# EpicOne1/grad_traj_optimization

Hardware: AMD Instinct MI355X
Metric: cost+grad evals/sec (batched trajectories) (higher is better)
Workload: dtype f64

## Files before the change

### grad_traj_optimization_amd/csrc/gtop_kernels.hip

```cpp

#include "gtop_wave_kernel.h"

#ifdef GTOP_CONSISTENT_TU
template <typename MM> using GtopModeOf = GtopConsistent<MM>;
#define GTOP_LAUNCHER(name) name##_consistent
constexpr bool kReferenceObject = false;
#else
template <typename MM> using GtopModeOf = MM;
#define GTOP_LAUNCHER(name) name
constexpr bool kReferenceObject = true;
#endif

namespace {

constexpr int kWaveMinw3From = 3072;

template <typename R, typename MM>
using WaveKernelFn = void (*)(const R *, const R *, const R *, const R *, int, int, int, int, int, int,
                              const GtopKernelArgs<R>, const GtopWaveConsts<R>, const MM, const GtopSetupConsts<R>);

template <typename R, bool WIDE, int SPL, int NT, int MINW, typename MM, bool LONG, int NW = 1>
static WaveKernelFn<R, MM> pick_body(bool colli, bool dyn) {
  if (!colli) {
    if constexpr (kIsCons<MM>) return nullptr;
    else return gtop_eval_wave_kernel<R, WIDE, SPL, NT, false, MINW, MM, false, LONG, NW>;
  }
  if (dyn) return gtop_eval_wave_kernel<R, WIDE, SPL, NT, true, (MINW < 3 ? 3 : MINW), MM, true, LONG, NW>;
  return gtop_eval_wave_kernel<R, WIDE, SPL, NT, true, MINW, MM, false, LONG, NW>;
}

template <typename R, bool WIDE, typename MM>
static WaveKernelFn<R, MM> pick_geometry(const GtopEvalPlan &p, int B, bool colli, bool dyn) {
  constexpr bool MMA = kIsMma<MM>;
  if (p.is_long) return pick_body<R, WIDE, 6, 1, 3, MM, true>(colli, dyn);
  if (p.spl == 30) {
    if constexpr (MMA) return nullptr;
    else return pick_body<R, WIDE, 30, 1, 3, MM, false>(colli, dyn);
  }
  if (p.spl == 10) {
    if constexpr (MMA) return nullptr;
    else return pick_body<R, WIDE, 10, 1, 3, MM, false>(colli, dyn);
  }
  if constexpr (!MMA) {
    if (p.nw == 2) return pick_body<R, WIDE, 3, 1, 2, MM, false, 2>(colli, dyn);
  }
  if (p.spl == 3) {
    if constexpr (!MMA && !(WIDE && sizeof(R) == 8)) {
      if (B >= kWaveMinw3From) return pick_body<R, WIDE, 3, 1, 3, MM, false>(colli, dyn);
    }
    return pick_body<R, WIDE, 3, 1, 2, MM, false>(colli, dyn);
  }
  if (p.nt == 2) {
    if constexpr (MMA) {
      if (dyn) return nullptr;
      if constexpr (kIsCons<MM>) {
        return colli ? gtop_eval_wave_kernel<R, WIDE, 6, 2, true, 3, MM, false, false, 1> : nullptr;
      } else {
        return colli ? gtop_eval_wave_kernel<R, WIDE, 6, 2, true, 3, MM, false, false, 1>
                     : gtop_eval_wave_kernel<R, WIDE, 6, 2, false, 3, MM, false, false, 1>;
      }
    } else {
      return pick_body<R, WIDE, 6, 2, 3, MM, false>(colli, dyn);
    }
  }
  return pick_body<R, WIDE, 6, 1, 3, MM, false>(colli, dyn);
}

template <bool WIDE, int SPL, int NT, typename MM, bool LONG>
static WaveKernelFn<double, MM> pick_body_moving(bool dyn) {
  if (dyn) return gtop_eval_wave_kernel<double, WIDE, SPL, NT, true, 3, MM, true, LONG, 1>;
  return gtop_eval_wave_kernel<double, WIDE, SPL, NT, true, 3, MM, false, LONG, 1>;
// ... 20 lines not shown
template <typename R> static bool has_collision_term(const GtopKernelArgs<R> &args) {
  return !((args.wc < (R)0 ? -args.wc : args.wc) < (R)1e-4);
}
template <typename MM> static GtopModeOf<MM> mode_args(const MM &st) {
  GtopModeOf<MM> w;
  static_cast<MM &>(w) = st;
  return w;
}

template <typename R, typename MM>
static hipError_t launch_wave(const GtopKernelArgs<R> &args, const MM &st, const GtopEvalPlan &plan, bool dyn,
                              hipStream_t stream) {
  constexpr bool MMA = kIsMma<MM>;
  constexpr bool MOV = kIsMov<MM>;
  if (args.B <= 0) return hipSuccess;
  GtopKernelArgs<R> wa = args;
  if (wa.step == 1) wa.ws = (R)0;
  const bool colli = has_collision_term(wa);
  dyn = dyn && wa.step == 2;
  const bool wide = !gtop_field_is_narrow(wa.nx, wa.ny, wa.nz, sizeof(R));
  WaveKernelFn<R, MM> kern;
  if constexpr (MOV) {
    if constexpr (!kIsCons<MM>) {
      using Base = typename MovingBase<MM>::type;
      if (!colli) return launch_wave<R, Base>(args, static_cast<const Base &>(st), plan, dyn, stream);
    }
    kern = wide ? pick_geometry_moving<true, MM>(plan, dyn) : pick_geometry_moving<false, MM>(plan, dyn);
  } else if constexpr (MMA && sizeof(R) == 4) {
    if (wide) return hipErrorInvalidValue;
    kern = pick_geometry<R, false, MM>(plan, wa.B, colli, dyn);
  } else {
    kern = wide ? pick_geometry<R, true, MM>(plan, wa.B, colli, dyn) : pick_geometry<R, false, MM>(plan, wa.B, colli, dyn);
  }
  if (!kern) return hipErrorInvalidValue;
  const size_t smem = gtop_wave_lds_bytes(plan, wa.m, MMA ? sizeof(double) : sizeof(R), MMA);
  if (smem > 160u * 1024u) return hipErrorInvalidValue;
  if (smem > 64u * 1024u) {
    hipError_t e = hipFuncSetAttribute(reinterpret_cast<const void *>(kern), hipFuncAttributeMaxDynamicSharedMemorySize,
                                       (int)smem);
    if (e != hipSuccess) return e;
  }
  const int n = 9 * (wa.m - 1);
  const long long per_launch = (long long)kMaxGroupsPerLaunch * plan.nt;
  if (MMA && wa.B > per_launch) return hipErrorInvalidValue;
  for (long long b0 = 0; b0 < args.B; b0 += per_launch) {
    GtopKernelArgs<R> s = wa;
    s.B = (int)((args.B - b0) < per_launch ? (args.B - b0) : per_launch);
    s.x = wa.x + (size_t)b0 * n;
    s.Df = wa.Df + (size_t)b0 * 18;
    s.T = wa.T + (size_t)b0 * wa.t_stride;
    s.cost = wa.cost ? wa.cost + b0 : nullptr;
    s.grad = wa.grad ? wa.grad + (size_t)b0 * n : nullptr;
    const int groups = (s.B + plan.nt - 1) / plan.nt;
    const int grid = 8 * ((groups + 7) / 8);
    MM sst = st;
    if constexpr (MOV) {
      if (sst.mk.t0) sst.mk.t0 += (size_t)b0 * (size_t)sst.mk.t0_stride;
    }
    hipLaunchKernelGGL(kern, dim3(grid), dim3(64 * plan.nw), smem, stream, s.x, s.Df, s.T, s.sdf, s.B, s.m, s.t_stride, s.nx, s.ny,
                       s.nz, s, GtopWaveConsts<R>{}, sst, GtopSetupConsts<R>{});
    hipError_t e = hipGetLastError();
    if (e != hipSuccess) return e;
  }
  return hipSuccess;
}

}


template <typename R>
hipError_t GTOP_LAUNCHER(gtop_launch_eval)(const GtopKernelArgs<R> &args, const GtopEvalPlan &plan, bool dyn, hipStream_t stream) {
  if (kReferenceObject && plan.consistent && has_collision_term(args)) return gtop_launch_eval_consistent<R>(args, plan, dyn, stream);
  return launch_wave<R, GtopModeOf<GtopNoMma>>(args, mode_args(GtopNoMma{}), plan, dyn, stream);
}

template <template <typename> class Moving = GtopMoving, typename Base>
static Moving<Base> moving_kernel_args(const Base &st, const GtopMovingArgs &mov) {
  Moving<Base> mm;
  static_cast<Base &>(mm) = st;
  mm.mk = GtopMovK{mov.rows, mov.t0, mov.nbox, mov.t0_stride};
  return mm;
}
hipError_t GTOP_LAUNCHER(gtop_launch_eval_moving)(const GtopKernelArgs<double> &args, const GtopEvalPlan &plan, bool dyn,
                                                  const GtopMovingArgs &mov, hipStream_t stream) {
  if (!mov.rows || mov.nbox < 1 || mov.nbox > GTOP_MOVING_MAX_BOXES) return hipErrorInvalidValue;
  if (kReferenceObject && plan.consistent && has_collision_term(args)) return gtop_launch_eval_moving_consistent(args, plan, dyn, mov, stream);
  if (mov.poly)
    return launch_wave<double, GtopModeOf<GtopMovingPoly<GtopNoMma>>>(args, mode_args(moving_kernel_args<GtopMovingPoly>(GtopNoMma{}, mov)), plan, dyn, stream);
  return launch_wave<double, GtopModeOf<GtopMoving<GtopNoMma>>>(args, mode_args(moving_kernel_args(GtopNoMma{}, mov)), plan, dyn, stream);
}
hipError_t GTOP_LAUNCHER(gtop_launch_eval_mma_moving)(const GtopKernelArgs<double> &args, const GtopMmaState &st,
                                                      const GtopEvalPlan &plan, bool dyn, const GtopMovingArgs &mov,
                                                      hipStream_t stream) {
  if (!mov.rows || mov.nbox < 1 || mov.nbox > GTOP_MOVING_MAX_BOXES) return hipErrorInvalidValue;
  if (plan.nt != 1) return hipErrorInvalidValue;
  if (kReferenceObject && plan.consistent && has_collision_term(args)) return gtop_launch_eval_mma_moving_consistent(args, st, plan, dyn, mov, stream);
  if (mov.poly)
    return launch_wave<double, GtopModeOf<GtopMovingPoly<GtopMmaState>>>(args, mode_args(moving_kernel_args<GtopMovingPoly>(st, mov)), plan, dyn, stream);
  return launch_wave<double, GtopModeOf<GtopMoving<GtopMmaState>>>(args, mode_args(moving_kernel_args(st, mov)), plan, dyn, stream);
}

hipError_t GTOP_LAUNCHER(gtop_launch_eval_mma)(const GtopKernelArgs<double> &args, const GtopMmaState &st,
                                               const GtopEvalPlan &plan, bool dyn, hipStream_t stream) {
  if (plan.nw != 1 || plan.spl == 30 || plan.spl == 10 || (plan.nt != 1 && !(plan.nt == 2 && plan.spl == 6 && !plan.is_long))) return hipErrorInvalidValue;
  if (kReferenceObject && plan.consistent && has_collision_term(args)) return gtop_launch_eval_mma_consistent(args, st, plan, dyn, stream);
  return launch_wave<double, GtopModeOf<GtopMmaState>>(args, mode_args(st), plan, dyn, stream);
}
hipError_t GTOP_LAUNCHER(gtop_launch_eval_mma)(const GtopKernelArgs<float> &args, const GtopMmaState &st,
                                               const GtopEvalPlan &plan, bool dyn, hipStream_t stream) {
  if (plan.nw != 1 || plan.spl == 30 || plan.spl == 10 || (plan.nt != 1 && !(plan.nt == 2 && plan.spl == 6 && !plan.is_long))) return hipErrorInvalidValue;
  if (kReferenceObject && plan.consistent && has_collision_term(args)) return gtop_launch_eval_mma_consistent(args, st, plan, dyn, stream);
  return launch_wave<float, GtopModeOf<GtopMmaState>>(args, mode_args(st), plan, dyn, stream);
}
// ... 27 lines not shown
```

### grad_traj_optimization_amd/csrc/gtop_wave_kernel.h

```cpp
#ifndef GTOP_WAVE_KERNEL_H_
#define GTOP_WAVE_KERNEL_H_
#include <type_traits>

#include "gtop_device_common.h"
#include "gtop_edt_lookup.h"
#include "gtop_kernels.h"

namespace {

#if defined(GTOP_STAMPS) && defined(GTOP_CONSISTENT_TU)
#undef GTOP_STAMPS
#endif
#ifdef GTOP_STAMPS
__device__ unsigned long long g_gtop_stamps[4096][16];
#if GTOP_STAMPS == 2
#define GTOP_STAMP_WANTED(i) ((i) == 0 || (i) == 11)
#else
#define GTOP_STAMP_WANTED(i) true
#endif
#define GTOP_STAMP(i)                                                                          \
  do {                                                                                         \
    if (GTOP_STAMP_WANTED(i)) {                                                                \
      unsigned long long t_;                                                                   \
      __builtin_amdgcn_sched_barrier(0);                                                       \
// ... 484 lines not shown
    q[k][4] = (K.k7 * V - K.k15 * P - A) * iT4;
    q[k][5] = (K.k6 * P - K.k3 * V + (C)0.5 * A) * iT5;
  }
}

template <typename C>
__device__ __forceinline__ C gtop_jerk_term(const C (&q)[3][6], C T, C wj, const GtopWaveConsts<C> &K, C (&g)[3][3]) {
  const C T2 = T * T, T3 = T2 * T, T4 = T2 * T2, T5 = T4 * T;
  const C Q33 = K.q36 * T, Q34 = K.q72 * T2, Q35 = K.q120 * T3, Q44 = K.q192 * T3, Q45 = K.q360 * T4, Q55 = K.q720 * T5;
  const C wj2 = wj + wj;
  C jc = (C)0;
#pragma unroll
  for (int k = 0; k < 3; ++k) {
    const C c3 = q[k][3], c4 = q[k][4], c5 = q[k][5];
    const C q3 = Q33 * c3 + Q34 * c4 + Q35 * c5;
    const C q4 = Q34 * c3 + Q44 * c4 + Q45 * c5;
    const C q5 = Q35 * c3 + Q45 * c4 + Q55 * c5;
    jc += c3 * q3 + c4 * q4 + c5 * q5;
    g[k][0] = wj2 * q3; g[k][1] = wj2 * q4; g[k][2] = wj2 * q5;
  }
  return wj * jc;
}

struct GtopNoMma {};
template <typename Base> struct GtopMoving : Base {
  GtopMovK mk;
};
template <typename Base> struct GtopMovingPoly : Base {
  GtopMovK mk;
};
template <typename MM> constexpr bool kIsMov = false;
template <typename Base> constexpr bool kIsMov<GtopMoving<Base>> = true;
template <typename Base> constexpr bool kIsMov<GtopMovingPoly<Base>> = true;
template <typename MM> constexpr bool kIsMovPoly = false;
template <typename Base> constexpr bool kIsMovPoly<GtopMovingPoly<Base>> = true;
template <typename MM> constexpr bool kIsMma = std::is_base_of<GtopMmaState, MM>::value;
template <typename Base> struct GtopConsistent : Base {};
template <typename MM> constexpr bool kIsCons = false;
template <typename Base> constexpr bool kIsCons<GtopConsistent<Base>> = true;
template <typename Base> constexpr bool kIsMov<GtopConsistent<Base>> = kIsMov<Base>;
template <typename Base> constexpr bool kIsMovPoly<GtopConsistent<Base>> = kIsMovPoly<Base>;
template <typename R, bool WIDE, typename MM, int SPL, int MINW, bool DYN, bool LONG>
constexpr int gtop_wave_budget() {
  if (kIsCons<MM> && kIsMovPoly<MM> && kIsMma<MM> && DYN && SPL == 6 && !LONG) return 1;
  return ((kIsMma<MM> && SPL == 6) || DYN || kIsMov<MM> || ((WIDE || LONG) && sizeof(R) == 8 && SPL >= 6) ||
          (sizeof(R) == 4 && SPL >= 6))
             ? 2
             : MINW;
}

template <typename R, bool WIDE, int SPL, int NT, bool COLLI, int MINW, typename MM = GtopNoMma, bool DYN = false,
          bool LONG = false, int NW = 1>
__global__ void __launch_bounds__(64 * NW) __attribute__((amdgpu_waves_per_eu(gtop_wave_budget<R, WIDE, MM, SPL, MINW, DYN, LONG>())))
gtop_eval_wave_kernel(const R *__restrict__ arg_x, const R *__restrict__ arg_Df, const R *__restrict__ arg_T,
                      const R *__restrict__ arg_sdf, int arg_B, int arg_m, int arg_t_stride, int arg_nx, int arg_ny,
                      int arg_nz, const GtopKernelArgs<R> arg_rest, const GtopWaveConsts<R> K, const MM st,
                      const GtopSetupConsts<R> KD) {
  constexpr bool MMA = kIsMma<MM>;
  constexpr bool MOV = kIsMov<MM>;
  constexpr bool CONS = kIsCons<MM>;
  static_assert(!CONS || COLLI, "the consistent gradient differs in the sample loop only");
  static_assert(!MMA || NT == 1 || (SPL == 6 && !LONG), "the optimizer loop: one trajectory per wavefront, or two at five lanes per segment");
  using In = typename std::conditional<MMA, double, R>::type;
  GtopKernelArgs<R> a = arg_rest;
  a.x = arg_x; a.Df = arg_Df; a.T = arg_T; a.sdf = arg_sdf;
  a.B = arg_B; a.m = arg_m; a.t_stride = arg_t_stride;
  a.nx = arg_nx; a.ny = arg_ny; a.nz = arg_nz;
  constexpr int LPS = kSamples / SPL;
  constexpr int SPW = 64 / LPS;
  constexpr int kStride = gtop_tile_stride(SPL, NW);
  constexpr int kMVc = gtop_mma_rows(SPL, NT);
  static_assert(SPL == 3 || SPL == 6 || SPL == 10 || SPL == 30, "10 or 5 lanes per segment; three or one with as many trajectories per wavefront as fit");
  constexpr bool MANY = SPL == 30 || SPL == 10;
  static_assert(!MANY || (NT == 1 && !LONG && !MMA && NW == 1 && MINW >= 3), "one lane per segment: plain evaluation, one sample (pair) at a time");
  static_assert(SPL == 3 || MINW >= 3, "six samples per lane: one (pair) at a time only");
  static_assert(NT == 1 || NT == 2, "one or two trajectories per wavefront");
  static_assert(!LONG || (SPL == 6 && NT == 1), "more than 12 segments: five lanes per segment, one trajectory");
  static_assert(!DYN || (COLLI && MINW >= 3), "the velocity/acceleration block lives in the sample loop, one sample at a time");
  static_assert(NW == 1 || (NW == 2 && SPL == 3 && NT == 1 && !LONG && !MMA), "two wavefronts per trajectory: plain evaluation at ten lanes per segment");
  static_assert(!MOV || (COLLI && MINW >= 3 && !kIsF32<R> && (SPL == 3 || SPL == 6) && NW == 1),
                "the moving-obstacle term: fp64, in the sample loop, one sample at a time, ten or five lanes per segment");
  extern __shared__ __align__(16) unsigned char smem_raw[];
  R *tile = reinterpret_cast<R *>(smem_raw);
  GTOP_STAMP(0);
  GTOP_STAMP_HWID();
  const int lane = NW == 2 ? (int)(threadIdx.x & 63u) : (int)threadIdx.x;
  const int wave = NW == 2 ? (int)(threadIdx.x >> 6) : 0;
  const int m = a.m, ndp = 3 * m - 3, n = 3 * ndp;
  if constexpr (LONG) __builtin_assume(m > SPW);
  else __builtin_assume(m >= 2 && NT * m <= NW * SPW);
  __builtin_assume(lane >= 0 && lane < 64);
  const int tstride = LONG ? gtop_tile_stride_long(m) : kStride;
  const int kMV = LONG ? gtop_mma_rows_long(n) : kMVc;
  const int nchunks = LONG ? (m + SPW - 1) / SPW : 1;
  constexpr int kTileRows = gtop_tile_rows(LONG);
  GTOP_STAMP(1);

  const int nt = MANY ? SPW / m : NT;
  const int ngroups = (a.B + nt - 1) / nt;
  const int per_xcd = (ngroups + 7) >> 3;
  const int grp_raw = ((int)blockIdx.x & 7) * per_xcd + ((int)blockIdx.x >> 3);
  const bool grp_ok = grp_raw < ngroups;
  const int grp = grp_ok ? grp_raw : ngroups - 1;
  const int b0 = grp * nt;

  const int slot_w = lane / LPS, li = lane - slot_w * LPS;
  const int slot = wave * SPW + slot_w;
  int tl = 0, s = slot;
  if constexpr (MANY) {
    tl = (int)(((unsigned)slot * (unsigned)((65536 + m - 1) / m)) >> 16);
    s -= tl * m;
  } else if constexpr (NT == 2) {
    tl = s >= m;
    s -= tl * m;
  }
  bool seg_ok = grp_ok & (slot_w < SPW) & (slot < nt * m) & (b0 + tl < a.B);
  if (!seg_ok) { tl = 0; s = 0; }

  unsigned long long t_launch = 0ull;
  int npass = 1;
  if constexpr (MMA) {
    t_launch = wall_clock64();
    npass = st.iters;
  }
  [[maybe_unused]] double *mv = nullptr;
  [[maybe_unused]] const int kState = LONG ? 0 : gtop_state_doubles(false, kMVc, 0);
  [[maybe_unused]] GtopMmaVecs mvecs[NT] = {};
  [[maybe_unused]] GtopMmaScalars msc[NT] = {};
  [[maybe_unused]] bool mma_live[NT] = {};
  if constexpr (MMA) {
    mv = reinterpret_cast<double *>(tile) + kTileRows * tstride + gtop_grad_rows(LONG, kMV);
#pragma unroll
    for (int t = 0; t < NT; ++t) {
    double *mvt = mv + t * kState;
    const int bt = b0 + t;
    mvecs[t] = GtopMmaVecs{mvt, mvt + kMV, mvt + 2 * kMV, mvt + 3 * kMV, mvt + 4 * kMV, mvt + 5 * kMV, mvt + 6 * kMV,
                           mvt + 7 * kMV, mvt + kMV};
    mma_live[t] = grp_ok & (bt < a.B);
    if (mma_live[t]) {
      const size_t o = (size_t)bt * n;
      const double *Df64 = reinterpret_cast<const double *>(a.Df), *T64 = reinterpret_cast<const double *>(a.T);
      if (lane < 18) mvt[kStateVecs * kMV + lane] = Df64[(size_t)bt * 18 + lane];
      if constexpr (LONG) {
        for (int j = lane; j < m; j += 64) mvt[kStateVecs * kMV + kDfVals + j] = T64[(size_t)bt * a.t_stride + j];
      } else {
        if (lane < m) mvt[kStateVecs * kMV + kDfVals + lane] = T64[(size_t)bt * a.t_stride + lane];
      }
      if (st.x0_init) {
        msc[t] = GtopMmaScalars{1.0, 0.0, 0.0, 0.0, 0.0, 0, 0, 0};
        for (int j = lane; j < n; j += 64) {
          const double lo = st.lb[o + j], hi = st.ub[o + j];
          double v = st.x0_init[o + j];
          v = v < lo ? lo : (v > hi ? hi : v);
          mvt[j] = v; mvt[kMV + j] = v; mvt[2 * kMV + j] = v; mvt[3 * kMV + j] = v;
          mvt[4 * kMV + j] = 0.0;
          mvt[5 * kMV + j] = (isinf(lo) || isinf(hi)) ? 1.0 : 0.5 * (hi - lo);
          mvt[6 * kMV + j] = lo;
          mvt[7 * kMV + j] = hi;
        }
      } else {
      msc[t] = gtop_mma_load_scalars(st, bt);
      for (int j = lane; j < n; j += 64) {
        mvt[j] = st.x[o + j];
        mvt[kMV + j] = st.xcur[o + j];
        mvt[2 * kMV + j] = st.xprev[o + j];
        mvt[3 * kMV + j] = st.xprevprev[o + j];
        mvt[4 * kMV + j] = st.dfdx[o + j];
        mvt[5 * kMV + j] = st.sigma[o + j];
        mvt[6 * kMV + j] = st.lb[o + j];
        mvt[7 * kMV + j] = st.ub[o + j];
      }
      }
    }
    }
    __builtin_amdgcn_fence(__ATOMIC_RELEASE, "wavefront");
    __builtin_amdgcn_wave_barrier();
  }
  [[maybe_unused]] double mov_t0 = 0.0;
  if constexpr (MOV) {
    if (st.mk.t0) mov_t0 = st.mk.t0[(size_t)(b0 + tl) * (size_t)st.mk.t0_stride];
  }
  for (int pass = 0; pass < npass; ++pass) {
  const R *xsrc = a.x;
  if constexpr (MMA) {
    bool running = false;
#pragma unroll
    for (int t = 0; t < NT; ++t) running |= mma_live[t] && msc[t].state < 3;
    if (!running) break;
    if (st.max_ticks > 0 && pass > 0 && (long long)(wall_clock64() - t_launch) > st.max_ticks) {
#pragma unroll
      for (int t = 0; t < NT; ++t)
        if (mma_live[t] && msc[t].state < 3) msc[t].state = GTOP_MMA_MAXTIME_REACHED;
      break;
    }
  }
  [[maybe_unused]] R cost_run = (R)0;
  constexpr int kRounds = (LONG || MANY) ? 1 : (NT * 9 * (NW * SPW / NT - 1) + 64 * NW - 1) / (64 * NW);
  const int tid = NW == 2 ? (int)threadIdx.x : lane;
  int offA[kRounds], offB[kRounds];
  bool okq[kRounds];
  bool cost_lane = false;
  [[maybe_unused]] double mov_seg = mov_t0;
  [[maybe_unused]] int mov_upto = 0;
  for (int ch = 0; ch < nchunks; ++ch) {
  if constexpr (LONG) {
    s = ch * SPW + slot_w;
    seg_ok = grp_ok & (slot_w < SPW) & (s < m);
    if (!seg_ok) s = 0;
  }
  const In *xb, *dfb, *Tb;
  if constexpr (MMA) {
    const double *mvl = mv + tl * kState;
    xb = mvl + kMV;
    dfb = mvl + kStateVecs * kMV;
    Tb = mvl + kStateVecs * kMV + kDfVals;
  } else {
    xb = xsrc + (size_t)b0 * n + tl * n;
    dfb = a.Df + (size_t)b0 * 18 + tl * 18;
    Tb = a.T + (size_t)b0 * a.t_stride + tl * a.t_stride;
  }
  const R T = (R)Tb[s];
  if constexpr (MOV) {
    constexpr int kPre = NT == 2 ? SPW / 2 : SPW;
    const int target = seg_ok ? s : mov_upto;
#pragma unroll
    for (int j = 0; j < kPre; ++j) {
      const int jj = mov_upto + j;
      const bool take = jj < target;
      const double Tj = (double)Tb[take ? jj : 0];
      mov_seg = take ? mov_seg + Tj : mov_seg;
    }
    mov_upto = target > mov_upto ? target : mov_upto;
  }
  const bool first = s == 0, last = s + 1 == m;
  const In *p0 = first ? dfb : xb + 3 * (s - 1);
  const In *p1 = last ? dfb + 3 : xb + 3 * s;
  const int st0 = first ? 6 : ndp, st1 = last ? 6 : ndp;
  R w0[3][3], w1[3][3];
#pragma unroll
  for (int k = 0; k < 3; ++k) {
#pragma unroll
    for (int i = 0; i < 3; ++i) {
      w0[k][i] = (R)p0[k * st0 + i];
      w1[k][i] = (R)p1[k * st1 + i];
    }
  }

#pragma unroll
  for (int r = 0; r < ((LONG || MANY) ? 0 : kRounds); ++r) {
    const int qi = tid + 64 * NW * r;
    int tq = 0, i = qi;
    if constexpr (NT == 2) {
      tq = i >= n;
      i -= tq * n;
    }
    okq[r] = grp_ok & (qi < NT * n) & (b0 + tq < a.B);
    const int axis = (i >= ndp) + (i >= 2 * ndp), c = i - axis * ndp;
    const int wpt = c / 3 + 1, der = c - 3 * (wpt - 1);
    const int rowB = axis * 6 + 2 * der;
    const int sA = tq * m + wpt - 1;
    offA[r] = okq[r] ? (rowB + 1) * kStride + sA * LPS : 0;
    offB[r] = okq[r] ? rowB * kStride + (sA + 1) * LPS : 0;
  }
  const int cs = lane - 48;
  const int ct = NT == 2 ? cs >> 3 : 0, csi = NT == 2 ? cs & 7 : cs;
  cost_lane = !LONG & !MANY & (wave == NW - 1) & (cs >= 0) & (csi < m);
  if (cost_lane) offA[kRounds - 1] = 18 * kStride + (ct * m + csi) * LPS;
  const R ws = a.ws;
  const R wc = a.wc;
  ExpConsts expk;
  R pen_d0 = a.d0, pen_inv_r = a.inv_r, pen_alpha = a.alpha, pen_gd = -a.alpha_over_r;
  MapBox<R> mapbox = {{a.lo[0], a.lo[1], a.lo[2]}, {a.hi[0], a.hi[1], a.hi[2]}};
  IndexBox ibox;
  if constexpr (kIsF32<R>) ibox = IndexBox{{a.idx_origin[0], a.idx_origin[1], a.idx_origin[2]}, a.idx_half, a.idx_rinv};
  else ibox = IndexBox{{(double)a.origin[0], (double)a.origin[1], (double)a.origin[2]}, 0.5 * (double)a.res, (double)a.res_inv};
  if constexpr (COLLI && !kIsF32<R> && MINW <= 2 && !MMA) {
    expk.pin();
  }
#if defined(GTOP_STAMPS) && GTOP_STAMPS != 2
  GTOP_STAMP(2);
  asm volatile("s_waitcnt vmcnt(0)" ::: "memory");
  GTOP_STAMP(3);
#endif
  const R T2 = T * T;
  const R iT = fast_rcp(T), iT3 = iT * iT * iT, iT4 = iT3 * iT, iT5 = iT4 * iT;
  const R dt = T * (R)(1.0 / 30.0);
  const R wdt = wc * dt;
  R q[3][6];
  [[maybe_unused]] double qd[kIsF32<R> ? 3 : 1][6];
  const GtopWaveConsts<double> &KC = gtop_setup_consts(K, KD);
  if constexpr (kIsF32<R>) {
    gtop_form_coefficients(qd, (double)T, KC, w0, w1);
#pragma unroll
    for (int k = 0; k < 3; ++k)
#pragma unroll
      for (int c = 0; c < 6; ++c) q[k][c] = (R)qd[k][c];
  } else {
    gtop_form_coefficients(q, T, K, w0, w1);
  }
  R acc[kRedVals];
  auto jerk_init = [&]() {
    const R wj = (seg_ok & (li == 0)) ? ws : (R)0;
    R g[3][3], jcost;
    if constexpr (kIsF32<R>) {
      double gdd[3][3];
      jcost = (R)gtop_jerk_term(qd, (double)T, (double)wj, KC, gdd);
#pragma unroll
      for (int k = 0; k < 3; ++k)
#pragma unroll
        for (int i = 0; i < 3; ++i) g[k][i] = (R)gdd[k][i];
    } else {
      jcost = gtop_jerk_term(q, T, wj, K, g);
    }
#pragma unroll
    for (int k = 0; k < 3; ++k) {
      acc[6 * k + 0] = (R)0; acc[6 * k + 1] = (R)0; acc[6 * k + 2] = (R)0;
      acc[6 * k + 3] = g[k][0]; acc[6 * k + 4] = g[k][1]; acc[6 * k + 5] = g[k][2];
    }
    acc[18] = jcost;
  };

  if constexpr (COLLI) {
    using TT = double;
    const TT Tt = (TT)T;
    TT dtt;
    if constexpr (kIsF32<R>) dtt = Tt * (1.0 / 30.0);
    else dtt = (TT)dt;
    const bool tiny_T = T < (R)0.0301;
    const bool any_tiny = __ballot(tiny_T) != 0ull;
    auto tiny_dt = [&]() {
      TT Tq = Tt;
      asm volatile("" : "+v"(Tq));
      return Tq / (TT)30.0;
    };
    const R aw_all = pen_alpha * wdt;
    auto sample_time = [&](int j, TT &t, R &awj, R &sdt, [[maybe_unused]] R &wdj) {
      t = (TT)(li + j * LPS) * dtt + (TT)1e-3;
      awj = aw_all;
      sdt = dt;
      if constexpr (CONS) wdj = wdt;
      if (any_tiny) {
        if (tiny_T) {
          const TT dtq = tiny_dt();
          t = (TT)1e-3;
          for (int i = 0; i < li + j * LPS; ++i) t += dtq;
          awj = (t < Tt) ? pen_alpha * (wc * (R)dtq) : (R)0;
          sdt = (t < Tt) ? (R)dtq : (R)0;
          if constexpr (CONS) wdj = (t < Tt) ? wc * (R)dtq : (R)0;
          t = (t < Tt) ? t : (TT)1e-3;
        }
      }
    };
    constexpr int NTS = (MINW <= 2) ? SPL : 1;
    TT ts[NTS];
    R aw[NTS];
    [[maybe_unused]] R sdts[NTS];
    [[maybe_unused]] R wds[NTS];
    if constexpr (MINW <= 2) {
#pragma unroll
      for (int j = 0; j < SPL; ++j) {
        ts[j] = (TT)(li + j * LPS) * dtt + (TT)1e-3;
        aw[j] = aw_all;
        sdts[j] = dt;
        if constexpr (CONS) wds[j] = wdt;
      }
      if (any_tiny) {
        if (tiny_T) {
          const TT dtq = tiny_dt();
          TT t = (TT)1e-3;
          int i = 0;
#pragma unroll
          for (int j = 0; j < SPL; ++j) {
            for (; i < li + j * LPS; ++i) t += dtq;
            ts[j] = (t < Tt) ? t : (TT)1e-3;
            aw[j] = (t < Tt) ? pen_alpha * (wc * (R)dtq) : (R)0;
            sdts[j] = (t < Tt) ? (R)dtq : (R)0;
            if constexpr (CONS) wds[j] = (t < Tt) ? wc * (R)dtq : (R)0;
          }
        }
      }
    }
    constexpr int CH = (MINW <= 2) ? SPL : 1;
    constexpr int kUnrollJ = (SPL <= 3 && MINW <= 2) ? SPL : 1;
#ifndef GTOP_ASM_LOADS
#define GTOP_ASM_LOADS 1
#endif
    constexpr bool ASMLD = GTOP_ASM_LOADS && !kIsF32<R> && !WIDE && MINW <= 2 && SPL == 3 && !MMA;
    if constexpr (kIsF32<R> && SPL % 2 == 0) {
      jerk_init();
      float cq[18];
#pragma unroll
      for (int k = 0; k < 3; ++k)
#pragma unroll
        for (int c = 0; c < 6; ++c) cq[6 * k + c] = (float)q[k][c];
      f2 acc2[kRedVals];
#pragma unroll
      for (int v = 0; v < kRedVals; ++v) acc2[v] = (f2){(float)acc[v], 0.0f};
#pragma unroll 1
      for (int jj = 0; jj < SPL; jj += 2) {
        TT tA, tB;
        R awA, awB, sdA, sdB, wdA, wdB;
        sample_time(jj, tA, awA, sdA, wdA);
        sample_time(jj + 1, tB, awB, sdB, wdB);
        sample_pair_f32<DYN, WIDE, CONS>(reinterpret_cast<const GtopKernelArgs<float> &>(a), ibox, qd, cq, tA, tB,
                                   DYN ? sdA != (R)0 : awA != (R)0, DYN ? sdB != (R)0 : awB != (R)0, (float)wdt,
                                   (float)dt, acc2);
      }
#pragma unroll
      for (int v = 0; v < kRedVals; ++v) acc[v] = (R)(acc2[v].x + acc2[v].y);
    } else {
    if constexpr (MINW > 2) jerk_init();
#pragma unroll kUnrollJ
    for (int j0 = 0; j0 < SPL; j0 += CH) {
      R vels[CH][3];
      [[maybe_unused]] R accs[CH][3];
      SdfTap<R> taps[CH];
      gtop_d2 raw[ASMLD ? CH : 1][4];
      if constexpr (MINW > 2) sample_time(j0, ts[0], aw[0], sdts[0], wds[0]);
      constexpr bool kRareOut = CH == SPL;
      constexpr bool kLoadsFirst = CH == 1 && !LONG;
      [[maybe_unused]] float pmin[3], pmax[3];
      [[maybe_unused]] bool outs[CH];
      [[maybe_unused]] double pos_mov[3];
      auto position = [&](int k, TT t, TT t2, TT t3, TT t4, TT t5) {
        if constexpr (kIsF32<R>)
          return (float)(qd[k][0] + qd[k][1] * t + qd[k][2] * t2 + qd[k][3] * t3 + qd[k][4] * t4 + qd[k][5] * t5);
        else
          return (float)(q[k][0] + q[k][1] * t + q[k][2] * t2 + q[k][3] * t3 + q[k][4] * t4 + q[k][5] * t5);
      };
#pragma unroll
      for (int c = 0; c < CH; ++c) {
        const TT tt = ts[MINW <= 2 ? j0 + c : 0];
        const TT u2 = tt * tt, u3 = u2 * tt, u4 = u2 * u2, u5 = u4 * tt;
        const R t = (R)tt;
        const R t2 = t * t, t3 = t2 * t, t4 = t2 * t2;
        const R d2 = (R)2 * t, d3 = K.k3 * t2, d4 = (R)4 * t3, d5 = K.k5 * t4;
        double pos[3];
        [[maybe_unused]] float posf[3];
#pragma unroll
        for (int k = 0; k < 3; ++k) {
          const float pf = position(k, tt, u2, u3, u4, u5);
          pos[k] = (double)pf;
          posf[k] = pf;
          if constexpr (MOV) pos_mov[k] = pos[k];
          if constexpr (kRareOut) {
            pmin[k] = c == 0 ? pf : fminf(pmin[k], pf);
            pmax[k] = c == 0 ? pf : fmaxf(pmax[k], pf);
          }
          if constexpr (!kLoadsFirst) {
            vels[c][k] = round_through_float(q[k][1] + q[k][2] * d2 + q[k][3] * d3 + q[k][4] * d4 + q[k][5] * d5);
            if constexpr (DYN)
              accs[c][k] = round_through_float((R)2 * q[k][2] + K.k6 * q[k][3] * t + (R)12 * q[k][4] * t2 + (R)20 * q[k][5] * t3);
          }
        }
        if constexpr (ASMLD) taps[c] = sdf_issue_asm(a, ibox, pos[0], pos[1], pos[2], raw[c]);
        else taps[c] = sdf_issue<R, WIDE>(a, ibox, pos[0], pos[1], pos[2]);
        if constexpr (!kRareOut) {
          if constexpr (kIsF32<R>) outs[c] = out_of_map(a.lo_f, a.hi_f, posf[0], posf[1], posf[2]);
          else outs[c] = out_of_map(mapbox.lo, mapbox.hi, (R)pos[0], (R)pos[1], (R)pos[2]);
        }
      }
      bool any_out = false;
      if constexpr (kRareOut) {
        const bool lane_out = (pmin[0] < a.lo_f[0]) | (pmin[1] < a.lo_f[1]) | (pmin[2] < a.lo_f[2]) |
                              (pmax[0] > a.hi_f[0]) | (pmax[1] > a.hi_f[1]) | (pmax[2] > a.hi_f[2]);
        any_out = __ballot(lane_out) != 0ull;
      }
      if (j0 == 0) GTOP_STAMP(4);
      if constexpr (CH == SPL || kLoadsFirst) GTOP_PHASE_FENCE();
      if constexpr (kLoadsFirst) {
        const R t = (R)ts[0];
        const R t2 = t * t, t3 = t2 * t, t4 = t2 * t2;
        const R d2 = (R)2 * t, d3 = K.k3 * t2, d4 = (R)4 * t3, d5 = K.k5 * t4;
#pragma unroll
        for (int k = 0; k < 3; ++k) {
          vels[0][k] = round_through_float(q[k][1] + q[k][2] * d2 + q[k][3] * d3 + q[k][4] * d4 + q[k][5] * d5);
          if constexpr (DYN)
            accs[0][k] = round_through_float((R)2 * q[k][2] + K.k6 * q[k][3] * t + (R)12 * q[k][4] * t2 + (R)20 * q[k][5] * t3);
        }
      }
      if constexpr (MINW <= 2) jerk_init();
      R vns[CH], ivns[CH];
#pragma unroll
      for (int c = 0; c < CH; ++c) {
        const R *vel = vels[c];
        vns[c] = speed_sqrt(vel[0] * vel[0] + vel[1] * vel[1] + vel[2] * vel[2]) + K.eps;
        ivns[c] = quick_rcp(vns[c]);
      }
#if defined(GTOP_STAMPS) && GTOP_STAMPS != 2
      if (j0 == 0) {
        asm volatile("" ::"v"(vns[0]), "v"(ivns[CH - 1]), "v"(acc[18]), "v"(acc[3]));
        GTOP_STAMP(5);
        asm volatile("s_waitcnt vmcnt(0)" ::: "memory");
        GTOP_STAMP(6);
      }
#endif
      if constexpr (CH == SPL) GTOP_PHASE_FENCE();
#pragma unroll
      for (int c = 0; c < CH; ++c) {
        if constexpr (ASMLD) {
          if (CH - 1 - c == 2) gtop_wait_pairs<8>(raw[c], acc[3], acc[17]);
          else if (CH - 1 - c == 1) gtop_wait_pairs<4>(raw[c], acc[3], acc[17]);
          else gtop_wait_pairs<0>(raw[c], acc[3], acc[17]);
#pragma unroll
          for (int q = 0; q < 4; ++q) {
            taps[c].v[2 * q] = raw[c][q].x;
            taps[c].v[2 * q + 1] = raw[c][q].y;
          }
        }
        const TT tt = ts[MINW <= 2 ? j0 + c : 0];
        const R t = (R)tt;
        const R *vel = vels[c];
        const R t2 = t * t, t3 = t2 * t, t4 = t2 * t2, t5 = t4 * t;
        const R vn = vns[c], ivn = ivns[c];
        R g3[3];
        if constexpr (MOV)
          mov_min_boxes<kIsMovPoly<MM>>(taps[c], a, ibox, pos_mov, mov_seg + (double)tt, st.mk, !outs[c]);
        R dist = sdf_blend(taps[c], g3[0], g3[1], g3[2]);
        if constexpr (!kRareOut) {
          dist = outs[c] ? (R)-1 : dist;
        } else if (any_out) {
          const TT u2 = tt * tt, u3 = u2 * tt, u4 = u2 * u2, u5 = u4 * tt;
          const float pfx = position(0, tt, u2, u3, u4, u5), pfy = position(1, tt, u2, u3, u4, u5),
                      pfz = position(2, tt, u2, u3, u4, u5);
          bool is_out;
          if constexpr (kIsF32<R>) is_out = out_of_map(a.lo_f, a.hi_f, pfx, pfy, pfz);
          else is_out = out_of_map(mapbox.lo, mapbox.hi, (R)pfx, (R)pfy, (R)pfz);
          if (is_out) {
            dist = (R)-1;
            g3[0] = g3[1] = g3[2] = (R)0;
          }
        }
        const R e = penalty_exp((pen_d0 - dist) * pen_inv_r, expk);
        const R cdw = aw[MINW <= 2 ? j0 + c : 0] * e;
        const R cv = cdw * vn;
        acc[18] = gfma(cdw, vn, acc[18]);
        R f1;
        if constexpr (CONS) f1 = ((pen_gd * a.res_inv) * e) * (wds[MINW <= 2 ? j0 + c : 0] * vn);
        else f1 = ((pen_gd * a.res_inv) * e) * cv;
        if constexpr (!kRareOut) f1 = outs[c] ? (R)0 : f1;
        const R f2 = cdw * ivn;
        const R d2 = (R)2 * t, d3 = K.k3 * t2, d4 = (R)4 * t3, d5 = K.k5 * t4;
        [[maybe_unused]] R dw2[3], dw3[3];
        if constexpr (DYN) {
          const R sdt = sdts[MINW <= 2 ? j0 + c : 0];
          const R *acc3 = accs[c];
          R ev[3], ea[3];
#pragma unroll
          for (int k = 0; k < 3; ++k) {
            ev[k] = penalty_exp((gabs(vel[k]) - a.v0) * a.inv_r_v, expk);
            ea[k] = penalty_exp((gabs(acc3[k]) - a.a0) * a.inv_r_a, expk);
          }
          const R csum_dyn = a.alpha_v * ((ev[0] + ev[1]) + ev[2]) + a.alpha_a * ((ea[0] + ea[1]) + ea[2]);
          acc[18] = gfma(csum_dyn * vn, sdt, acc[18]);
          if constexpr (CONS) {
            const R call = csum_dyn * ivn;
#pragma unroll
            for (int k = 0; k < 3; ++k) {
              const R sv = (R)((vel[k] > (R)0) - (vel[k] < (R)0)), sa = (R)((acc3[k] > (R)0) - (acc3[k] < (R)0));
              dw2[k] = (a.gv_scale * ev[k] * sv * vn + call * vel[k]) * sdt;
              dw3[k] = (a.ga_scale * ea[k] * sa * vn) * sdt;
            }
          } else {
          const R clast = (a.alpha_v * ev[2] + a.alpha_a * ea[2]) * ivn;
#pragma unroll
          for (int k = 0; k < 3; ++k) {
            dw2[k] = (a.gv_scale * ev[k] * vn + clast * vel[k]) * sdt;
            dw3[k] = (a.ga_scale * ea[k] * vn) * sdt;
          }
          }
        }
#pragma unroll
        for (int k = 0; k < 3; ++k) {
          const R w1k = f1 * g3[k], w2k = f2 * vel[k];
          R *ak = acc + 6 * k;
          ak[0] = gfma(f1, g3[k], ak[0]);
          ak[1] = gfma(w1k, t, gfma(f2, vel[k], ak[1]));
          ak[2] = gfma(w1k, t2, gfma(w2k, d2, ak[2]));
          ak[3] = gfma(w1k, t3, gfma(w2k, d3, ak[3]));
          ak[4] = gfma(w1k, t4, gfma(w2k, d4, ak[4]));
          ak[5] = gfma(w1k, t5, gfma(w2k, d5, ak[5]));
          if constexpr (DYN) {
            ak[1] += dw2[k];
            ak[2] = gfma(dw2[k], d2, gfma(dw3[k], (R)2, ak[2]));
            ak[3] = gfma(dw2[k], d3, gfma(dw3[k] * K.k6, t, ak[3]));
            ak[4] = gfma(dw2[k], d4, gfma(dw3[k] * (R)12, t2, ak[4]));
            ak[5] = gfma(dw2[k], d5, gfma(dw3[k] * (R)20, t3, ak[5]));
          }
        }
      }
      if constexpr (CH != SPL) __builtin_amdgcn_sched_barrier(0);
    }
    }
  } else {
    (void)wdt; (void)pen_d0; (void)pen_inv_r; (void)pen_alpha; (void)pen_gd;
    jerk_init();
  }
#if defined(GTOP_STAMPS) && GTOP_STAMPS != 2
  asm volatile("" ::"v"(acc[0]), "v"(acc[5]), "v"(acc[11]), "v"(acc[17]), "v"(acc[18]));
  GTOP_STAMP(7);
#endif
  R jT3 = iT3, jT4 = iT4, jT5 = iT5;
  if constexpr (MINW > 2) {
    R iTb = iT;
    asm volatile("" : "+v"(iTb));
    jT3 = iTb * iTb * iTb; jT4 = jT3 * iTb; jT5 = jT4 * iTb;
  }
#pragma unroll
  for (int k = 0; k < 3; ++k) {
    R *g = acc + 6 * k;
    const R H3 = g[3] * jT3, H4 = g[4] * jT4, H5 = g[5] * jT5;
    const R ap = K.k10 * H3 - K.k15 * H4 + K.k6 * H5;
    const R o0 = g[0] - ap;
    const R o2 = g[1] + T * (K.k8 * H4 - K.k6 * H3 - K.k3 * H5);
    const R o3 = T * (K.k7 * H4 - (R)4 * H3 - K.k3 * H5);
    const R o4 = (R)0.5 * g[2] + T2 * (K.k1p5 * H4 - K.k1p5 * H3 - (R)0.5 * H5);
    const R o5 = T2 * ((R)0.5 * H3 - H4 + (R)0.5 * H5);
    g[0] = o0; g[1] = ap; g[2] = o2; g[3] = o3; g[4] = o4; g[5] = o5;
  }
  if constexpr (LONG) {
    if (seg_ok) {
      const int col = s * LPS + li;
#pragma unroll
      for (int v = 0; v < 18; ++v) tile[v * tstride + col] = acc[v];
      cost_run += acc[18];
    }
  } else {
  if (lane < LPS * SPW) {
#pragma unroll
    for (int v = 0; v < kRedVals; ++v) tile[v * kStride + wave * (LPS * SPW) + lane] = acc[v];
  }
  }
  GTOP_STAMP(8);
  GTOP_STAMP(9);
  }
  if constexpr (NW == 2) {
    __syncthreads();
  } else {
    __builtin_amdgcn_fence(__ATOMIC_RELEASE, "wavefront");
    __builtin_amdgcn_wave_barrier();
  }
  R csum_seg = (R)0;
  R *gl = tile + kTileRows * tstride;
  if constexpr (LONG) {
    for (int qi = lane; qi < n; qi += 64) {
      const int axis = (qi >= ndp) + (qi >= 2 * ndp), c = qi - axis * ndp;
      const int wpt = c / 3 + 1, der = c - 3 * (wpt - 1);
      const int rowB = axis * 6 + 2 * der;
      const R sa = tree_sum<R, LPS>(tile + (rowB + 1) * tstride + (wpt - 1) * LPS),
              sb = tree_sum<R, LPS>(tile + rowB * tstride + wpt * LPS);
      if constexpr (MMA) gl[qi] = (sa + sb) + K.eps;
      else if (grp_ok) a.grad[(size_t)b0 * n + qi] = (sa + sb) + K.eps;
    }
    const R ctot = gtop_wave_sum(cost_run) + (R)1e-3;
    if constexpr (MMA) {
      __builtin_amdgcn_fence(__ATOMIC_RELEASE, "wavefront");
      __builtin_amdgcn_wave_barrier();
      gtop_mma_update_core(st, mvecs[0], msc[0], n, lane, (double)ctot, static_cast<const R *>(gl));
      __builtin_amdgcn_fence(__ATOMIC_RELEASE, "wavefront");
      __builtin_amdgcn_wave_barrier();
    } else {
      if (grp_ok & (lane == 0)) a.cost[b0] = ctot;
    }
  } else if constexpr (MANY) {
    const int ntn = nt * n, ntasks = ntn + nt;
    const unsigned inv_n = (unsigned)(((1u << 24) + (unsigned)n - 1u) / (unsigned)n);
    for (int r0 = 0; r0 < ntasks; r0 += 64) {
      const int qi = r0 + lane;
      if (qi < ntn) {
        const int tq = (int)(((unsigned)qi * inv_n) >> 24);
        const int i = qi - tq * n;
        const int axis = (i >= ndp) + (i >= 2 * ndp), c = i - axis * ndp;
        const int wpt = c / 3 + 1, der = c - 3 * (wpt - 1);
        const int rowB = axis * 6 + 2 * der, sA = tq * m + wpt - 1;
        const R gq = (tree_sum<R, LPS>(tile + (rowB + 1) * kStride + sA * LPS) +
                      tree_sum<R, LPS>(tile + rowB * kStride + (sA + 1) * LPS)) + K.eps;
        if (grp_ok & (b0 + tq < a.B)) a.grad[(size_t)b0 * n + qi] = gq;
      } else if (qi < ntasks) {
        const int t = qi - ntn;
        const R *row = tile + 18 * kStride + t * m * LPS;
        R csum = tree_sum<R, LPS>(row);
        for (int sg = 1; sg < m; ++sg) csum += tree_sum<R, LPS>(row + sg * LPS);
        if (grp_ok & (b0 + t < a.B)) a.cost[b0 + t] = csum + (R)1e-3;
      }
    }
  } else {
#pragma unroll
  for (int r = 0; r < kRounds; ++r) {
    const R sa = tree_sum<R, LPS>(tile + offA[r]), sb = tree_sum<R, LPS>(tile + offB[r]);
    R gq = (sa + sb) + K.eps;
    asm volatile("" : "+v"(gq));
    if (r == kRounds - 1 && cost_lane) csum_seg = sa;
    if constexpr (MMA) {
      if (okq[r]) gl[lane + 64 * r] = gq;
    } else {
      if (okq[r]) a.grad[(size_t)b0 * n + tid + 64 * NW * r] = gq;
    }
  }
  {
    R cpart = cost_lane ? csum_seg : (R)0;
    cpart += gtop_dpp_move<0x111>(cpart);
    cpart += gtop_dpp_move<0x112>(cpart);
    cpart += gtop_dpp_move<0x114>(cpart);
    if constexpr (NT == 2 && MMA) {
      const unsigned long long u = __builtin_bit_cast(unsigned long long, (double)(cpart + (R)1e-3));
      __builtin_amdgcn_fence(__ATOMIC_RELEASE, "wavefront");
      __builtin_amdgcn_wave_barrier();
#pragma unroll
      for (int t = 0; t < 2; ++t) {
        const unsigned lo32 = (unsigned)__builtin_amdgcn_readlane((int)(unsigned)u, 55 + 8 * t);
        const unsigned hi32 = (unsigned)__builtin_amdgcn_readlane((int)(unsigned)(u >> 32), 55 + 8 * t);
        const double fcur = __builtin_bit_cast(double, ((unsigned long long)hi32 << 32) | lo32);
        if (mma_live[t]) gtop_mma_update_core(st, mvecs[t], msc[t], n, lane, fcur, static_cast<const R *>(gl) + t * n);
      }
      __builtin_amdgcn_fence(__ATOMIC_RELEASE, "wavefront");
      __builtin_amdgcn_wave_barrier();
    } else if constexpr (NT == 2) {
      if (grp_ok & (lane == 55)) a.cost[b0] = cpart + (R)1e-3;
      if (grp_ok & (lane == 63) & (b0 + 1 < a.B)) a.cost[b0 + 1] = cpart + (R)1e-3;
    } else if constexpr (NW * SPW > 8 && !MMA) {
      cpart += gtop_dpp_move<0x118>(cpart);
      if (grp_ok & (wave == NW - 1) & (lane == 63)) a.cost[b0] = cpart + (R)1e-3;
    } else if constexpr (MMA) {
      constexpr int kCostLane = SPW > 8 ? 63 : 55;
      if constexpr (SPW > 8) cpart += gtop_dpp_move<0x118>(cpart);
      const unsigned long long u = __builtin_bit_cast(unsigned long long, (double)(cpart + (R)1e-3));
      const unsigned lo32 = (unsigned)__builtin_amdgcn_readlane((int)(unsigned)u, kCostLane);
      const unsigned hi32 = (unsigned)__builtin_amdgcn_readlane((int)(unsigned)(u >> 32), kCostLane);
      const double fcur = __builtin_bit_cast(double, ((unsigned long long)hi32 << 32) | lo32);
      __builtin_amdgcn_fence(__ATOMIC_RELEASE, "wavefront");
      __builtin_amdgcn_wave_barrier();
      gtop_mma_update_core(st, mvecs[0], msc[0], n, lane, fcur, static_cast<const R *>(gl));
      __builtin_amdgcn_fence(__ATOMIC_RELEASE, "wavefront");
      __builtin_amdgcn_wave_barrier();
    } else {
      if (grp_ok & (lane == 55)) a.cost[b0] = cpart + (R)1e-3;
    }
  }
  }
  GTOP_STAMP(10);
#ifdef GTOP_STAMPS
  asm volatile("s_waitcnt vmcnt(0)" ::: "memory");
  GTOP_STAMP(11);
#endif
  }
  if constexpr (MMA) {
    __builtin_amdgcn_fence(__ATOMIC_RELEASE, "wavefront");
    __builtin_amdgcn_wave_barrier();
#pragma unroll
    for (int t = 0; t < NT; ++t) {
    if (mma_live[t]) {
      const double *mvt = mv + t * kState;
// ... 26 lines not shown
```

Before: 276.0 million.

## Precompute grid mapping on host and prefetch kernel-argument lines at entry

Moves per-group index arithmetic (groups per XCD, last group, byte offsets for x and T) from the kernel prologue to the host launcher, and drops the unused nx/ny/nz arguments. For one kernel variant it issues early scalar loads touching each 64-byte line of the kernel-argument block so later argument reads hit cache. It also simplifies the waypoint pointer setup in the non-MMA path and removes bounds checks that cannot fail when there is one trajectory per group. Several GTOP_MARK hooks are added; they appear undefined in the visible code, so the change relies on a definition elsewhere.

Result: faster. 280.0 million (median of 6 runs) (+1.5%).

```diff
diff --git a/grad_traj_optimization_amd/csrc/gtop_kernels.hip b/grad_traj_optimization_amd/csrc/gtop_kernels.hip
--- a/grad_traj_optimization_amd/csrc/gtop_kernels.hip
+++ b/grad_traj_optimization_amd/csrc/gtop_kernels.hip
@@ -16,7 +16,7 @@
 constexpr int kWaveMinw3From = 3072;
 
 template <typename R, typename MM>
-using WaveKernelFn = void (*)(const R *, const R *, const R *, const R *, int, int, int, int, int, int,
+using WaveKernelFn = void (*)(const R *, const R *, const R *, int, int, int, int, int, unsigned, unsigned, const R *,
                               const GtopKernelArgs<R>, const GtopWaveConsts<R>, const MM, const GtopSetupConsts<R>);
 
 template <typename R, bool WIDE, int SPL, int NT, int MINW, typename MM, bool LONG, int NW = 1>
@@ -143,13 +143,16 @@
     s.cost = wa.cost ? wa.cost + b0 : nullptr;
     s.grad = wa.grad ? wa.grad + (size_t)b0 * n : nullptr;
     const int groups = (s.B + plan.nt - 1) / plan.nt;
-    const int grid = 8 * ((groups + 7) / 8);
+    const int per_xcd = (groups + 7) / 8;
+    const int grid = 8 * per_xcd;
+    const unsigned x_grp_bytes = (unsigned)((size_t)plan.nt * (size_t)n * sizeof(R));
+    const unsigned T_grp_bytes = (unsigned)((size_t)plan.nt * (size_t)wa.t_stride * sizeof(R));
     MM sst = st;
     if constexpr (MOV) {
       if (sst.mk.t0) sst.mk.t0 += (size_t)b0 * (size_t)sst.mk.t0_stride;
     }
-    hipLaunchKernelGGL(kern, dim3(grid), dim3(64 * plan.nw), smem, stream, s.x, s.Df, s.T, s.sdf, s.B, s.m, s.t_stride, s.nx, s.ny,
-                       s.nz, s, GtopWaveConsts<R>{}, sst, GtopSetupConsts<R>{});
+    hipLaunchKernelGGL(kern, dim3(grid), dim3(64 * plan.nw), smem, stream, s.x, s.Df, s.T, s.B, s.m, s.t_stride, per_xcd,
+                       groups - 1, x_grp_bytes, T_grp_bytes, s.sdf, s, GtopWaveConsts<R>{}, sst, GtopSetupConsts<R>{});
     hipError_t e = hipGetLastError();
     if (e != hipSuccess) return e;
   }
diff --git a/grad_traj_optimization_amd/csrc/gtop_wave_kernel.h b/grad_traj_optimization_amd/csrc/gtop_wave_kernel.h
--- a/grad_traj_optimization_amd/csrc/gtop_wave_kernel.h
+++ b/grad_traj_optimization_amd/csrc/gtop_wave_kernel.h
@@ -560,10 +560,10 @@
 template <typename R, bool WIDE, int SPL, int NT, bool COLLI, int MINW, typename MM = GtopNoMma, bool DYN = false,
           bool LONG = false, int NW = 1>
 __global__ void __launch_bounds__(64 * NW) __attribute__((amdgpu_waves_per_eu(gtop_wave_budget<R, WIDE, MM, SPL, MINW, DYN, LONG>())))
-gtop_eval_wave_kernel(const R *__restrict__ arg_x, const R *__restrict__ arg_Df, const R *__restrict__ arg_T,
-                      const R *__restrict__ arg_sdf, int arg_B, int arg_m, int arg_t_stride, int arg_nx, int arg_ny,
-                      int arg_nz, const GtopKernelArgs<R> arg_rest, const GtopWaveConsts<R> K, const MM st,
-                      const GtopSetupConsts<R> KD) {
+gtop_eval_wave_kernel(const R *__restrict__ arg_x, const R *__restrict__ arg_Df, const R *__restrict__ arg_T, int arg_B,
+                      int arg_m, int arg_t_stride, int arg_per_xcd, int arg_last_grp, unsigned arg_x_grp_bytes,
+                      unsigned arg_T_grp_bytes, const R *__restrict__ arg_sdf, const GtopKernelArgs<R> arg_rest,
+                      const GtopWaveConsts<R> K, const MM st, const GtopSetupConsts<R> KD) {
   constexpr bool MMA = kIsMma<MM>;
   constexpr bool MOV = kIsMov<MM>;
   constexpr bool CONS = kIsCons<MM>;
@@ -573,7 +573,6 @@
   GtopKernelArgs<R> a = arg_rest;
   a.x = arg_x; a.Df = arg_Df; a.T = arg_T; a.sdf = arg_sdf;
   a.B = arg_B; a.m = arg_m; a.t_stride = arg_t_stride;
-  a.nx = arg_nx; a.ny = arg_ny; a.nz = arg_nz;
   constexpr int LPS = kSamples / SPL;
   constexpr int SPW = 64 / LPS;
   constexpr int kStride = gtop_tile_stride(SPL, NW);
@@ -592,8 +591,24 @@
   R *tile = reinterpret_cast<R *>(smem_raw);
   GTOP_STAMP(0);
   GTOP_STAMP_HWID();
-  const int lane = NW == 2 ? (int)(threadIdx.x & 63u) : (int)threadIdx.x;
-  const int wave = NW == 2 ? (int)(threadIdx.x >> 6) : 0;
+  GTOP_MARK(1);
+  constexpr bool kLone = COLLI && !kIsF32<R> && !WIDE && MINW <= 2 && SPL == 3 && !kIsMma<MM> && !LONG;
+  static_assert(!kLone || (64 + sizeof(GtopKernelArgs<R>) + sizeof(GtopWaveConsts<R>) > 0x200 &&
+                           64 + sizeof(GtopKernelArgs<R>) + sizeof(GtopWaveConsts<R>) <= 0x240),
+                "the entry touches the nine 64-byte lines of the kernel-argument block: leading arguments, a, K");
+  [[maybe_unused]] unsigned kpre[9];
+  unsigned wg_id = blockIdx.x, thr_id = threadIdx.x;
+  if constexpr (kLone) {
+    const auto kp = __builtin_amdgcn_kernarg_segment_ptr();
+    asm volatile("s_load_dword %0, %11, 0x0\n\ts_load_dword %1, %11, 0x40\n\ts_load_dword %2, %11, 0x80\n\t"
+                 "s_load_dword %3, %11, 0xc0\n\ts_load_dword %4, %11, 0x100\n\ts_load_dword %5, %11, 0x140\n\t"
+                 "s_load_dword %6, %11, 0x180\n\ts_load_dword %7, %11, 0x1c0\n\ts_load_dword %8, %11, 0x200"
+                 : "=&s"(kpre[0]), "=&s"(kpre[1]), "=&s"(kpre[2]), "=&s"(kpre[3]), "=&s"(kpre[4]), "=&s"(kpre[5]),
+                   "=&s"(kpre[6]), "=&s"(kpre[7]), "=&s"(kpre[8]), "+s"(wg_id), "+v"(thr_id)
+                 : "s"(kp));
+  }
+  const int lane = NW == 2 ? (int)(thr_id & 63u) : (int)thr_id;
+  const int wave = NW == 2 ? (int)(thr_id >> 6) : 0;
   const int m = a.m, ndp = 3 * m - 3, n = 3 * ndp;
   if constexpr (LONG) __builtin_assume(m > SPW);
   else __builtin_assume(m >= 2 && NT * m <= NW * SPW);
@@ -605,12 +620,13 @@
   GTOP_STAMP(1);
 
   const int nt = MANY ? SPW / m : NT;
-  const int ngroups = (a.B + nt - 1) / nt;
-  const int per_xcd = (ngroups + 7) >> 3;
-  const int grp_raw = ((int)blockIdx.x & 7) * per_xcd + ((int)blockIdx.x >> 3);
-  const bool grp_ok = grp_raw < ngroups;
-  const int grp = grp_ok ? grp_raw : ngroups - 1;
+  const int per_xcd = arg_per_xcd, last_grp = arg_last_grp;
+  const int grp_raw = ((int)wg_id & 7) * per_xcd + ((int)wg_id >> 3);
+  const bool grp_ok = grp_raw <= last_grp;
+  const int grp = grp_ok ? grp_raw : last_grp;
   const int b0 = grp * nt;
+  [[maybe_unused]] const uint64_t x_grp_off = (uint64_t)(uint32_t)grp * (uint64_t)arg_x_grp_bytes;
+  [[maybe_unused]] const uint64_t T_grp_off = (uint64_t)(uint32_t)grp * (uint64_t)arg_T_grp_bytes;
 
   const int slot_w = lane / LPS, li = lane - slot_w * LPS;
   const int slot = wave * SPW + slot_w;
@@ -622,7 +638,8 @@
     tl = s >= m;
     s -= tl * m;
   }
-  bool seg_ok = grp_ok & (slot_w < SPW) & (slot < nt * m) & (b0 + tl < a.B);
+  const bool row_ok = (NT == 1 && !MANY) ? true : (b0 + tl < a.B);
+  bool seg_ok = grp_ok & (slot_w < SPW) & (slot < nt * m) & row_ok;
   if (!seg_ok) { tl = 0; s = 0; }
 
   unsigned long long t_launch = 0ull;
@@ -704,7 +721,7 @@
   }
   [[maybe_unused]] R cost_run = (R)0;
   constexpr int kRounds = (LONG || MANY) ? 1 : (NT * 9 * (NW * SPW / NT - 1) + 64 * NW - 1) / (64 * NW);
-  const int tid = NW == 2 ? (int)threadIdx.x : lane;
+  const int tid = NW == 2 ? (int)thr_id : lane;
   int offA[kRounds], offB[kRounds];
   bool okq[kRounds];
   bool cost_lane = false;
@@ -723,9 +740,9 @@
     dfb = mvl + kStateVecs * kMV;
     Tb = mvl + kStateVecs * kMV + kDfVals;
   } else {
-    xb = xsrc + (size_t)b0 * n + tl * n;
-    dfb = a.Df + (size_t)b0 * 18 + tl * 18;
-    Tb = a.T + (size_t)b0 * a.t_stride + tl * a.t_stride;
+    xb = reinterpret_cast<const R *>(reinterpret_cast<const char *>(xsrc) + x_grp_off) + tl * n;
+    dfb = a.Df + (size_t)(uint32_t)b0 * 18 + tl * 18;
+    Tb = reinterpret_cast<const R *>(reinterpret_cast<const char *>(a.T) + T_grp_off) + tl * a.t_stride;
   }
   const R T = (R)Tb[s];
   if constexpr (MOV) {
@@ -741,19 +758,37 @@
     mov_upto = target > mov_upto ? target : mov_upto;
   }
   const bool first = s == 0, last = s + 1 == m;
-  const In *p0 = first ? dfb : xb + 3 * (s - 1);
-  const In *p1 = last ? dfb + 3 : xb + 3 * s;
-  const int st0 = first ? 6 : ndp, st1 = last ? 6 : ndp;
   R w0[3][3], w1[3][3];
-#pragma unroll
-  for (int k = 0; k < 3; ++k) {
-#pragma unroll
-    for (int i = 0; i < 3; ++i) {
-      w0[k][i] = (R)p0[k * st0 + i];
-      w1[k][i] = (R)p1[k * st1 + i];
-    }
-  }
-
+  if constexpr (MMA) {
+    const In *p0 = first ? dfb : xb + 3 * (s - 1);
+    const In *p1 = last ? dfb + 3 : xb + 3 * s;
+    const int st0 = first ? 6 : ndp, st1 = last ? 6 : ndp;
+#pragma unroll
+    for (int k = 0; k < 3; ++k) {
+#pragma unroll
+      for (int i = 0; i < 3; ++i) {
+        w0[k][i] = (R)p0[k * st0 + i];
+        w1[k][i] = (R)p1[k * st1 + i];
+      }
+    }
+  } else {
+    const In *pm = xb + 3 * s, *dfe = dfb + 3;
+    const In *p0 = first ? dfe : pm;
+    const In *p1 = last ? dfe : pm;
+    const int st0 = first ? 6 : ndp, st1 = last ? 6 : ndp;
+#pragma unroll
+    for (int k = 0; k < 3; ++k) {
+#pragma unroll
+      for (int i = 0; i < 3; ++i) {
+        w0[k][i] = (R)p0[i - 3];
+        w1[k][i] = (R)p1[i];
+      }
+      p0 += st0;
+      p1 += st1;
+    }
+  }
+
+  GTOP_MARK(2);
 #pragma unroll
   for (int r = 0; r < ((LONG || MANY) ? 0 : kRounds); ++r) {
     const int qi = tid + 64 * NW * r;
@@ -762,7 +797,7 @@
       tq = i >= n;
       i -= tq * n;
     }
-    okq[r] = grp_ok & (qi < NT * n) & (b0 + tq < a.B);
+    okq[r] = grp_ok & (qi < NT * n) & (NT == 1 || b0 + tq < a.B);
     const int axis = (i >= ndp) + (i >= 2 * ndp), c = i - axis * ndp;
     const int wpt = c / 3 + 1, der = c - 3 * (wpt - 1);
     const int rowB = axis * 6 + 2 * der;
@@ -785,11 +820,16 @@
   if constexpr (COLLI && !kIsF32<R> && MINW <= 2 && !MMA) {
     expk.pin();
   }
+  GTOP_MARK(3);
 #if defined(GTOP_STAMPS) && GTOP_STAMPS != 2
   GTOP_STAMP(2);
   asm volatile("s_waitcnt vmcnt(0)" ::: "memory");
   GTOP_STAMP(3);
 #endif
+  if constexpr (kLone)
+    asm volatile("s_waitcnt lgkmcnt(0) ; entry lines %0 %1 %2 %3 %4 %5 %6 %7 %8"
+                 : "+s"(kpre[0]), "+s"(kpre[1]), "+s"(kpre[2]), "+s"(kpre[3]), "+s"(kpre[4]), "+s"(kpre[5]), "+s"(kpre[6]),
+                   "+s"(kpre[7]), "+s"(kpre[8]));
   const R T2 = T * T;
   const R iT = fast_rcp(T), iT3 = iT * iT * iT, iT4 = iT3 * iT, iT5 = iT4 * iT;
   const R dt = T * (R)(1.0 / 30.0);
@@ -829,6 +869,7 @@
   };
 
   if constexpr (COLLI) {
+    GTOP_MARK(4);
     using TT = double;
     const TT Tt = (TT)T;
     TT dtt;
@@ -920,6 +961,7 @@
     if constexpr (MINW > 2) jerk_init();
 #pragma unroll kUnrollJ
     for (int j0 = 0; j0 < SPL; j0 += CH) {
+      GTOP_MARK(5);
       R vels[CH][3];
       [[maybe_unused]] R accs[CH][3];
       SdfTap<R> taps[CH];
@@ -976,6 +1018,7 @@
       }
       if (j0 == 0) GTOP_STAMP(4);
       if constexpr (CH == SPL || kLoadsFirst) GTOP_PHASE_FENCE();
+      GTOP_MARK(6);
       if constexpr (kLoadsFirst) {
         const R t = (R)ts[0];
         const R t2 = t * t, t3 = t2 * t, t4 = t2 * t2;
@@ -1004,6 +1047,7 @@
       }
 #endif
       if constexpr (CH == SPL) GTOP_PHASE_FENCE();
+      GTOP_MARK(7);
 #pragma unroll
       for (int c = 0; c < CH; ++c) {
         if constexpr (ASMLD) {
@@ -1108,6 +1152,7 @@
   asm volatile("" ::"v"(acc[0]), "v"(acc[5]), "v"(acc[11]), "v"(acc[17]), "v"(acc[18]));
   GTOP_STAMP(7);
 #endif
+  GTOP_MARK(8);
   R jT3 = iT3, jT4 = iT4, jT5 = iT5;
   if constexpr (MINW > 2) {
     R iTb = iT;
@@ -1126,6 +1171,7 @@
     const R o5 = T2 * ((R)0.5 * H3 - H4 + (R)0.5 * H5);
     g[0] = o0; g[1] = ap; g[2] = o2; g[3] = o3; g[4] = o4; g[5] = o5;
   }
+  GTOP_MARK(9);
   if constexpr (LONG) {
     if (seg_ok) {
       const int col = s * LPS + li;
@@ -1148,6 +1194,7 @@
     __builtin_amdgcn_fence(__ATOMIC_RELEASE, "wavefront");
     __builtin_amdgcn_wave_barrier();
   }
+  GTOP_MARK(11);
   R csum_seg = (R)0;
   R *gl = tile + kTileRows * tstride;
   if constexpr (LONG) {
@@ -1206,6 +1253,7 @@
     }
   }
   {
+    GTOP_MARK(10);
     R cpart = cost_lane ? csum_seg : (R)0;
     cpart += gtop_dpp_move<0x111>(cpart);
     cpart += gtop_dpp_move<0x112>(cpart);
```
